# samuelkriegerbonini-dev/AstroBurst

Hardware: AMD Instinct MI355X
Metric: MPix/s sigma-clipped stack+stretch, 64x4096x4096 f32 (higher is better)
Workload: dtype f32

## Files before the change

### astroburst_amd/csrc/resample.hip

```cpp
#include "ab_common.hpp"
#include <algorithm>
#include <climits>
#include <cmath>

namespace {

__device__ __forceinline__ double cr_inner(double t) { return t * t * (1.5 * t - 2.5) + 1.0; }
__device__ __forceinline__ double cr_outer(double t) { return t * (t * (2.5 - 0.5 * t) - 4.0) + 2.0; }

__device__ __forceinline__ void catmull_weights(double f, double &w0, double &w1, double &w2, double &w3) {
    w0 = cr_outer(fabs(f + 1.0));
    w1 = cr_inner(fabs(f));
    w2 = cr_inner(fabs(f - 1.0));
    w3 = cr_outer(fabs(f - 2.0));
}

__device__ __forceinline__ int clamp_i32(int idx, int len) {
    return idx < 0 ? 0 : (idx >= len ? len - 1 : idx);
}

__device__ __forceinline__ float bicubic_taps(const float *__restrict__ src, int rows, int cols, int ld, int ix, int iy,
                                              double wx0, double wx1, double wx2, double wx3, double wy0, double wy1,
                                              double wy2, double wy3) {
    const int c0 = clamp_i32(ix - 1, cols), c1 = clamp_i32(ix, cols), c2 = clamp_i32(ix + 1, cols),
              c3 = clamp_i32(ix + 2, cols);
    const int r0 = clamp_i32(iy - 1, rows) * ld, r1 = clamp_i32(iy, rows) * ld, r2 = clamp_i32(iy + 1, rows) * ld,
              r3 = clamp_i32(iy + 2, rows) * ld;
    const double wy[4] = {wy0, wy1, wy2, wy3};
    const int rr[4] = {r0, r1, r2, r3};
    double val = 0.0;
#pragma unroll
    for (int j = 0; j < 4; ++j) {
        const float *row = src + rr[j];
        double row_val = (double)row[c0] * wx0;
        row_val += (double)row[c1] * wx1;
        row_val += (double)row[c2] * wx2;
        row_val += (double)row[c3] * wx3;
        const double t = row_val * wy[j];
        val = (j == 0) ? t : val + t;
    }
    return (float)val;
}

__device__ __forceinline__ float bicubic_taps_interior(const float *__restrict__ src, int ld, int ix, int iy, double wx0, double wx1,
                                                       double wx2, double wx3, double wy0, double wy1, double wy2, double wy3) {
    const float *p = src + (iy - 1) * ld + (ix - 1);
    const double wy[4] = {wy0, wy1, wy2, wy3};
    double val = 0.0;
#pragma unroll
    for (int j = 0; j < 4; ++j) {
        const float *row = p + j * ld;
        double row_val = (double)row[0] * wx0;
        row_val += (double)row[1] * wx1;
        row_val += (double)row[2] * wx2;
        row_val += (double)row[3] * wx3;
        const double t = row_val * wy[j];
        val = (j == 0) ? t : val + t;
    }
    return (float)val;
}

template <bool GUARD = false>
__device__ __forceinline__ float bicubic_sample(const float *__restrict__ src, int rows, int cols, int ld, double y, double x,
                                                bool sample = true) {
    const double xf = floor(x), yf = floor(y);
    double wx0, wx1, wx2, wx3, wy0, wy1, wy2, wy3;
    catmull_weights(x - xf, wx0, wx1, wx2, wx3);
    catmull_weights(y - yf, wy0, wy1, wy2, wy3);
    int ix = (int)xf, iy = (int)yf;
    if constexpr (GUARD) {
        if (x != x) ix = 0, wx0 = wx1 = wx2 = wx3 = 0.0;
        if (y != y) iy = 0, wy0 = wy1 = wy2 = wy3 = 0.0;
    }
    const bool interior = ix >= 1 && ix + 2 < cols && iy >= 1 && iy + 2 < rows;
    if (__all(interior || !sample)) {
        if (!sample) return 0.0f;
        return bicubic_taps_interior(src, ld, ix, iy, wx0, wx1, wx2, wx3, wy0, wy1, wy2, wy3);
    }
    if (!sample) return 0.0f;
    return bicubic_taps(src, rows, cols, ld, ix, iy, wx0, wx1, wx2, wx3, wy0, wy1, wy2, wy3);
}

__device__ __forceinline__ void xcd_band_piece(unsigned int &piece_x, unsigned int &piece_y) {
    piece_x = blockIdx.x;
    piece_y = blockIdx.y;
#ifndef AB_WARP_ROW_MAJOR
    if ((gridDim.x & 7u) != 0) {
        const unsigned int gx = gridDim.x, total = gx * gridDim.y, id = blockIdx.y * gx + blockIdx.x;
        const unsigned int c = id & 7u, k = id >> 3;
        unsigned int start = 0;
        for (unsigned int j = 0; j < c; ++j) start += (total - j + 7u) >> 3;
        const unsigned int t = start + k;
        piece_y = t / gx;
        piece_x = t - piece_y * gx;
    }
#endif
}

template <bool GUARD>
__global__ __launch_bounds__(256) void shift_kernel(const float *__restrict__ src, int rows, int cols, int ld, double dy,
                                                    double dx, float *__restrict__ out) {
    unsigned int piece_x, piece_y;
    xcd_band_piece(piece_x, piece_y);
    const int x = piece_x * 256 + threadIdx.x;
    const int y = piece_y;
    if (x >= cols) return;
    const double sy = (double)y + dy;
    const double sx = (double)x + dx;
    float r = 0.0f;
    if (!(sy < -0.5 || sy > (double)rows - 0.5 || sx < -0.5 || sx > (double)cols - 0.5))
        r = bicubic_sample<GUARD>(src, rows, cols, ld, sy, sx);
    out[(size_t)y * cols + x] = r;
}

__device__ __forceinline__ double cr_outer_fused(double t) { return t * (t * __builtin_fma(-0.5, t, 2.5) - 4.0) + 2.0; }
__device__ __forceinline__ void catmull_weights_fused(double f, double &w0, double &w1, double &w2, double &w3) {
    w0 = cr_outer_fused(fabs(f + 1.0));
    w1 = cr_inner(fabs(f));
    w2 = cr_inner(fabs(f - 1.0));
    w3 = cr_outer_fused(fabs(f - 2.0));
}

template <bool GUARD, bool NOLOAD = false, bool NOCVT = false>
__global__ __launch_bounds__(256) void warp_kernel(const float *__restrict__ src, int src_rows, int src_cols, double a,
                                                   double b, double tx, double c, double d, double ty, int out_rows,
                                                   int out_cols, float *__restrict__ out, int row0) {
#ifdef AB_WARP_WAVE_PRIO
    __builtin_amdgcn_s_setprio(AB_WARP_WAVE_PRIO);
#endif
    unsigned int piece_x, piece_y;
    xcd_band_piece(piece_x, piece_y);
    const int x0 = piece_x * 512 + threadIdx.x;
    const int y = piece_y + row0;
    const double yf = (double)y;
    float r[2];
    bool live[2];
#pragma unroll
    for (int u = 0; u < 2; ++u) {
        const int x = x0 + 256 * u;
        live[u] = x < out_cols;
        const double xf = (double)x;
        const double sx = a * xf + b * yf + tx;
        const double sy = c * xf + d * yf + ty;
        const double fx = floor(sx), fy = floor(sy);
        int ix, iy;
        asm("v_cvt_i32_f64 %0, %1" : "=v"(ix) : "v"(fx));
        asm("v_cvt_i32_f64 %0, %1" : "=v"(iy) : "v"(fy));
        bool in = live[u] && (unsigned)ix < (unsigned)(src_cols - 1) && (unsigned)iy < (unsigned)(src_rows - 1);
        if constexpr (GUARD) in = in && sx == sx && sy == sy;
        double wx0, wx1, wx2, wx3, wy0, wy1, wy2, wy3;
        catmull_weights_fused(sx - fx, wx0, wx1, wx2, wx3);
        catmull_weights_fused(sy - fy, wy0, wy1, wy2, wy3);
        const bool interior = ix >= 1 && ix + 2 < src_cols && iy >= 1 && iy + 2 < src_rows;
        r[u] = 0.0f;
        if constexpr (NOLOAD) {
            double val = 0.0;
            const double wy[4] = {wy0, wy1, wy2, wy3};
#pragma unroll
            for (int j = 0; j < 4; ++j) {
                float s0 = __int_as_float(0x3f800000 | ((ix + 4 * j) & 0xffff)), s1 = __int_as_float(0x3f800000 | ((ix + 4 * j + 1) & 0xffff)),
                      s2 = __int_as_float(0x3f800000 | ((iy + 4 * j + 2) & 0xffff)), s3 = __int_as_float(0x3f800000 | ((iy + 4 * j + 3) & 0xffff));
                double d0 = (double)s0, d1 = (double)s1, d2 = (double)s2, d3 = (double)s3;
                if constexpr (NOCVT) {
                    d0 = __longlong_as_double(0x3ff0000000000000ll | (long long)(unsigned)(ix + 4 * j));
                    d1 = __longlong_as_double(0x3ff0000000000000ll | (long long)(unsigned)(ix + 4 * j + 1));
                    d2 = __longlong_as_double(0x3ff0000000000000ll | (long long)(unsigned)(iy + 4 * j + 2));
                    d3 = __longlong_as_double(0x3ff0000000000000ll | (long long)(unsigned)(iy + 4 * j + 3));
                }
                double row_val = d0 * wx0;
                row_val += d1 * wx1;
                row_val += d2 * wx2;
                row_val += d3 * wx3;
                const double t = row_val * wy[j];
                val = (j == 0) ? t : val + t;
            }
            r[u] = in ? (float)val : 0.0f;
        } else if (__all(interior || !in)) {
            if (in) r[u] = bicubic_taps_interior(src, src_cols, ix, iy, wx0, wx1, wx2, wx3, wy0, wy1, wy2, wy3);
        } else if (in) {
            r[u] = bicubic_taps(src, src_rows, src_cols, src_cols, ix, iy, wx0, wx1, wx2, wx3, wy0, wy1, wy2, wy3);
        }
    }
#pragma unroll
    for (int u = 0; u < 2; ++u)
        if (live[u]) out[(size_t)piece_y * out_cols + x0 + 256 * u] = r[u];
}

__global__ __launch_bounds__(256) void resample_kernel(const float *__restrict__ src, int src_rows, int src_cols, double scale_y,
                                                       double scale_x, double half_shift_y, double half_shift_x, int out_cols,
                                                       float *__restrict__ out) {
    unsigned int piece_x, piece_y;
    xcd_band_piece(piece_x, piece_y);
    const int x = piece_x * 256 + threadIdx.x;
    const int y = piece_y;
    if (x >= out_cols) return;
    const double sy = (double)y * scale_y + half_shift_y;
    const double sx = (double)x * scale_x + half_shift_x;
    out[(size_t)y * out_cols + x] = bicubic_sample(src, src_rows, src_cols, src_cols, sy, sx);
}

}

int ab_resample_device(ab_ctx *ctx, const float *src, int64_t src_rows, int64_t src_cols, int64_t out_rows, int64_t out_cols,
                       float *out) {
    AB_HIP(ctx, hipSetDevice(ctx->device));
    if (out_rows == 0 || out_cols == 0) return ab_set_error(ctx, AB_ERR_INVALID, "Target dimensions must be > 0");
    if (out_rows == src_rows && out_cols == src_cols) {
        if (src != out) AB_HIP(ctx, hipMemcpyAsync(out, src, (size_t)src_rows * src_cols * sizeof(float), hipMemcpyDeviceToDevice, ctx->stream));
        return AB_OK;
    }
    AB_CHECK(ctx, src != out, "resample_image cannot run in place");
    AB_CHECK(ctx, src_rows > 0 && src_cols > 0, "resample_image: empty source");
    AB_CHECK(ctx, out_rows <= 65535 && out_rows * out_cols < (int64_t(1) << 31) && src_rows * src_cols < (int64_t(1) << 31),
             "image of %lld x %lld needs a tiled launch (not in this build)", (long long)out_rows, (long long)out_cols);
    const double scale_y = (double)src_rows / (double)out_rows, scale_x = (double)src_cols / (double)out_cols;
    const dim3 grid((unsigned)((out_cols + 255) / 256), (unsigned)out_rows), block(256);
    hipLaunchKernelGGL(resample_kernel, grid, block, 0, ctx->stream, src, (int)src_rows, (int)src_cols, scale_y, scale_x,
                       (scale_y - 1.0) * 0.5, (scale_x - 1.0) * 0.5, (int)out_cols, out);
    AB_HIP(ctx, hipGetLastError());
    return AB_OK;
}

int ab_shift_device(ab_ctx *ctx, const float *src, int64_t rows, int64_t cols, int64_t src_ld, double dy, double dx, float *out) {
    AB_HIP(ctx, hipSetDevice(ctx->device));
    if (fabs(dy) < 1e-12 && fabs(dx) < 1e-12) {
        if (src != out)
            AB_HIP(ctx, hipMemcpy2DAsync(out, cols * sizeof(float), src, src_ld * sizeof(float), cols * sizeof(float), rows,
                                         hipMemcpyDeviceToDevice, ctx->stream));
        return AB_OK;
    }
    AB_CHECK(ctx, src != out, "shift_image_subpixel cannot run in place");
    AB_CHECK(ctx, rows <= 65535 && rows * src_ld < (int64_t(1) << 31),
             "image of %lld x %lld needs a tiled launch (not in this build)", (long long)rows, (long long)cols);
    const dim3 grid((unsigned)((cols + 255) / 256), (unsigned)rows), block(256);
    if (std::isfinite(dy) && std::isfinite(dx))
        hipLaunchKernelGGL(shift_kernel<false>, grid, block, 0, ctx->stream, src, (int)rows, (int)cols, (int)src_ld, dy, dx, out);
    else
        hipLaunchKernelGGL(shift_kernel<true>, grid, block, 0, ctx->stream, src, (int)rows, (int)cols, (int)src_ld, dy, dx, out);
    AB_HIP(ctx, hipGetLastError());
    return AB_OK;
}

int ab_warp_device(ab_ctx *ctx, const float *src, int64_t src_rows, int64_t src_cols, const double t[6], int64_t out_rows,
                   int64_t out_cols, float *out) {
    return ab_warp_rows_device(ctx, src, src_rows, src_cols, t, out_rows, out_cols, 0, out_rows, out);
}

constexpr long kWarpLdsKB = 0;
int ab_warp_rows_device(ab_ctx *ctx, const float *src, int64_t src_rows, int64_t src_cols, const double t[6], int64_t out_rows,
                        int64_t out_cols, int64_t row0, int64_t nrows, float *out) {
    AB_HIP(ctx, hipSetDevice(ctx->device));
    AB_CHECK(ctx, row0 >= 0 && nrows >= 0 && row0 + nrows <= out_rows, "row band [%lld, %lld) leaves the %lld output rows", (long long)row0,
             (long long)(row0 + nrows), (long long)out_rows);
    if (nrows == 0) return AB_OK;
    AB_CHECK(ctx, src != out, "warp_image cannot run in place");
    AB_CHECK(ctx, out_rows <= 65535 && out_rows * out_cols < (int64_t(1) << 31) && src_rows * src_cols < (int64_t(1) << 31),
             "image of %lld x %lld needs a tiled launch (not in this build)", (long long)out_rows, (long long)out_cols);
    const dim3 grid((unsigned)((out_cols + 511) / 512), (unsigned)nrows), block(256);
#ifdef AB_DEV_ABLATION
    static const int ablate = ab_dev_env("AB_ABLATE_WARP") ? atoi(ab_dev_env("AB_ABLATE_WARP")) : 0;
    if (ablate == 1) return AB_OK;
    if (ablate == 3) {
        const dim3 g2((unsigned)((out_cols + 511) / 512), (unsigned)nrows);
        hipLaunchKernelGGL((warp_kernel<false, true, true>), g2, dim3(256), 0, ctx->stream, src, (int)src_rows, (int)src_cols, t[0], t[1], t[2], t[3],
                           t[4], t[5], (int)out_rows, (int)out_cols, out, (int)row0);
        return AB_OK;
    }
    if (ablate == 2) {
        const dim3 g2((unsigned)((out_cols + 511) / 512), (unsigned)nrows);
        hipLaunchKernelGGL((warp_kernel<false, true>), g2, dim3(256), 0, ctx->stream, src, (int)src_rows, (int)src_cols, t[0], t[1], t[2], t[3],
                           t[4], t[5], (int)out_rows, (int)out_cols, out, (int)row0);
        return AB_OK;
    }
#endif
    bool tame = true;
    for (int i = 0; i < 6; ++i) tame = tame && std::isfinite(t[i]) && fabs(t[i]) <= 1e150;
    static const unsigned warp_lds = [] {
        const char *e = ab_dev_env("AB_WARP_LDS_KB");
        const long kb = e ? atol(e) : kWarpLdsKB;
        return (unsigned)(kb < 0 ? 0 : (kb > 64 ? 64 : kb)) * 1024u;
    }();
    if (tame)
        hipLaunchKernelGGL(warp_kernel<false>, grid, block, warp_lds, ctx->stream, src, (int)src_rows, (int)src_cols, t[0], t[1], t[2], t[3],
                           t[4], t[5], (int)out_rows, (int)out_cols, out, (int)row0);
    else
        hipLaunchKernelGGL(warp_kernel<true>, grid, block, warp_lds, ctx->stream, src, (int)src_rows, (int)src_cols, t[0], t[1], t[2], t[3],
                           t[4], t[5], (int)out_rows, (int)out_cols, out, (int)row0);
    AB_HIP(ctx, hipGetLastError());
    return AB_OK;
}

extern "C" {

int ab_shift_image_subpixel(ab_ctx *ctx, const ab_plane *src, double dy, double dx, ab_plane_mut *out) try {
    if (!ctx) return AB_ERR_INVALID;
    AB_CHECK(ctx, src && out, "null plane");
    AB_CHECK(ctx, src->rows == out->rows && src->cols == out->cols, "shift_image_subpixel keeps the image dims");
    StagedPlane in;
    AB_TRY(ab_stage_in(ctx, src, &in));
    StagedOut so;
    int rc = ab_stage_out_begin(ctx, out, &so);
    if (rc == AB_OK) {
        rc = ab_shift_device(ctx, in.dptr, in.rows, in.cols, in.cols, dy, dx, so.dptr);
        if (rc == AB_OK)
            rc = ab_stage_out_finish(ctx, &so);
        else
            ab_stage_out_abort(ctx, &so);
    }
    ab_stage_release(ctx, &in);
    return rc;
} AB_CATCH(ctx)

int ab_warp_image_rows(ab_ctx *ctx, const ab_plane *src, const double transform[6], int64_t out_rows, int64_t row0, ab_plane_mut *out_band) try {
    if (!ctx) return AB_ERR_INVALID;
    AB_CHECK(ctx, src && out_band && transform && src->data && out_band->data, "null plane or transform");
    AB_CHECK(ctx, src->on_device && out_band->on_device, "ab_warp_image_rows takes device-resident planes");
    return ab_warp_rows_device(ctx, src->data, src->rows, src->cols, transform, out_rows, out_band->cols, row0, out_band->rows, out_band->data);
} AB_CATCH(ctx)

static void warp_source_rows(const double t[6], int64_t src_rows, int64_t src_cols, int64_t out_cols, int64_t row0, int64_t nrows,
                             int64_t *s0, int64_t *sn) {
    *s0 = 0;
    *sn = 0;
    if (nrows <= 0 || out_cols <= 0 || src_rows < 2 || src_cols < 2) return;
    for (int i = 0; i < 6; ++i)
        if (!std::isfinite(t[i]) || fabs(t[i]) > 1e150) {
            *sn = src_rows;
            return;
        }
    double lo = INFINITY, hi = -INFINITY;
    const double xs[2] = {0.0, (double)(out_cols - 1)}, ys[2] = {(double)row0, (double)(row0 + nrows - 1)};
    for (double xf : xs)
        for (double yf : ys) {
            const double sy = t[3] * xf + t[4] * yf + t[5];
            lo = std::min(lo, sy);
            hi = std::max(hi, sy);
        }
    const double last = (double)(src_rows - 2);
    if (!(hi >= 0.0) || !(floor(lo) <= last)) return;
    const int64_t f_lo = (int64_t)std::max(floor(lo), 0.0), f_hi = (int64_t)std::min(floor(hi), last);
    const int64_t a = std::max<int64_t>(f_lo - 1, 0), b = std::min<int64_t>(f_hi + 2, src_rows - 1);
    *s0 = a;
    *sn = b - a + 1;
}

int ab_warp_source_rows(const double transform[6], int64_t src_rows, int64_t src_cols, int64_t out_cols, int64_t row0, int64_t nrows,
                        int64_t *src_row0, int64_t *src_nrows) try {
    if (!transform || !src_row0 || !src_nrows || src_rows < 0 || src_cols < 0 || row0 < 0 || nrows < 0) return AB_ERR_INVALID;
    warp_source_rows(transform, src_rows, src_cols, out_cols, row0, nrows, src_row0, src_nrows);
    return AB_OK;
} AB_CATCH_NOCTX

int ab_shard_source_rows(const double *transforms, size_t n, int64_t src_rows, int64_t src_cols, int64_t out_rows, int64_t out_cols, int nranks,
                         int rank, int64_t *src_row0, int64_t *src_nrows) try {
    if ((!transforms && n) || !src_row0 || !src_nrows) return AB_ERR_INVALID;
    int64_t row0 = 0, nrows = 0;
    if (ab_shard_rows(out_rows, nranks, rank, &row0, &nrows) != AB_OK) return AB_ERR_INVALID;
    int64_t lo = INT64_MAX, hi = INT64_MIN;
    for (size_t i = 0; i < n; ++i) {
        int64_t s0 = 0, sn = 0;
        warp_source_rows(transforms + 6 * i, src_rows, src_cols, out_cols, row0, nrows, &s0, &sn);
        if (sn > 0) {
            lo = std::min(lo, s0);
            hi = std::max(hi, s0 + sn);
        }
    }
    *src_row0 = lo <= hi ? lo : 0;
    *src_nrows = lo <= hi ? hi - lo : 0;
    return AB_OK;
} AB_CATCH_NOCTX

int ab_warp_image_rows_from_band(ab_ctx *ctx, const ab_plane *src_band, int64_t src_row0, int64_t src_rows, const double transform[6],
                                 int64_t out_rows, int64_t row0, ab_plane_mut *out_band) try {
    if (!ctx) return AB_ERR_INVALID;
    AB_CHECK(ctx, src_band && out_band && transform && (out_band->rows == 0 || out_band->data), "null plane or transform");
    AB_CHECK(ctx, src_row0 >= 0 && src_band->rows >= 0 && src_row0 + src_band->rows <= src_rows, "source band [%lld, %lld) leaves the frame's %lld rows",
             (long long)src_row0, (long long)(src_row0 + src_band->rows), (long long)src_rows);
    if (out_band->rows == 0) return AB_OK;
    AB_CHECK(ctx, out_band->on_device && (src_band->rows == 0 || (src_band->data && src_band->on_device)), "ab_warp_image_rows_from_band takes device-resident planes");
    int64_t need0 = 0, need_n = 0;
    warp_source_rows(transform, src_rows, src_band->cols, out_band->cols, row0, out_band->rows, &need0, &need_n);
    AB_CHECK(ctx, need_n == 0 || (need0 >= src_row0 && need0 + need_n <= src_row0 + src_band->rows),
             "output rows [%lld, %lld) read source rows [%lld, %lld); the band holds [%lld, %lld)", (long long)row0, (long long)(row0 + out_band->rows),
             (long long)need0, (long long)(need0 + need_n), (long long)src_row0, (long long)(src_row0 + src_band->rows));
    const float *base = src_band->data ? src_band->data - src_row0 * src_band->cols : nullptr;
    if (!base) {
        base = out_band->data + 1;
    }
    return ab_warp_rows_device(ctx, base, src_rows, src_band->cols, transform, out_rows, out_band->cols, row0, out_band->rows, out_band->data);
} AB_CATCH(ctx)

int ab_warp_image(ab_ctx *ctx, const ab_plane *src, const double transform[6], ab_plane_mut *out) try {
    if (!ctx) return AB_ERR_INVALID;
    AB_CHECK(ctx, src && out && transform, "null plane or transform");
    StagedPlane in;
    AB_TRY(ab_stage_in(ctx, src, &in));
    StagedOut so;
    int rc = ab_stage_out_begin(ctx, out, &so);
    if (rc == AB_OK) {
        rc = ab_warp_device(ctx, in.dptr, in.rows, in.cols, transform, out->rows, out->cols, so.dptr);
        if (rc == AB_OK)
            rc = ab_stage_out_finish(ctx, &so);
        else
            ab_stage_out_abort(ctx, &so);
    }
    ab_stage_release(ctx, &in);
    return rc;
} AB_CATCH(ctx)

int ab_resample_image(ab_ctx *ctx, const ab_plane *src, ab_plane_mut *out) try {
    if (!ctx) return AB_ERR_INVALID;
    AB_CHECK(ctx, src && out, "null plane");
    if (out->rows == 0 || out->cols == 0) return ab_set_error(ctx, AB_ERR_INVALID, "Target dimensions must be > 0");
    StagedPlane in;
    AB_TRY(ab_stage_in(ctx, src, &in));
    StagedOut so;
    int rc = ab_stage_out_begin(ctx, out, &so);
    if (rc == AB_OK) {
        rc = ab_resample_device(ctx, in.dptr, in.rows, in.cols, out->rows, out->cols, so.dptr);
        if (rc == AB_OK)
            rc = ab_stage_out_finish(ctx, &so);
        else
            ab_stage_out_abort(ctx, &so);
    }
    ab_stage_release(ctx, &in);
    return rc;
} AB_CATCH(ctx)

}
```

Measured before the change: 112,300.

## Add multi-row warp kernel that shares source tap rows across adjacent outputs

Adds a warp kernel variant in which each thread computes K vertically adjacent output rows. When the affine map is close to identity in y, those outputs read overlapping 4x4 source neighbourhoods, so the kernel loads K+3 source rows once instead of 4K. The variant is selected when the transform is tame and near-unit in y, with a wave-uniform fallback to the per-pixel path. The intent is to cut redundant global loads and index math, at the cost of more registers per thread and fewer threads in the grid.

```diff
diff --git a/astroburst_amd/csrc/resample.hip b/astroburst_amd/csrc/resample.hip
--- a/astroburst_amd/csrc/resample.hip
+++ b/astroburst_amd/csrc/resample.hip
@@ -186,6 +186,99 @@
         if (live[u]) out[(size_t)piece_y * out_cols + x0 + 256 * u] = r[u];
 }
 
+template <int J>
+__device__ __forceinline__ double catmull_weight_fused(double f) {
+    if constexpr (J == 0) return cr_outer_fused(fabs(f + 1.0));
+    if constexpr (J == 1) return cr_inner(fabs(f));
+    if constexpr (J == 2) return cr_inner(fabs(f - 1.0));
+    return cr_outer_fused(fabs(f - 2.0));
+}
+
+template <int K>
+__global__ __launch_bounds__(256) void warp_kernel_shared(const float *__restrict__ src, int src_rows, int src_cols, double a, double b,
+                                                          double tx, double c, double d, double ty, int out_rows, int out_cols,
+                                                          float *__restrict__ out, int row0, int nrows) {
+    unsigned int piece_x, piece_y;
+    xcd_band_piece(piece_x, piece_y);
+    const int x = piece_x * 256 + threadIdx.x;
+    const int yb = piece_y * K;
+    const bool col_live = x < out_cols;
+    const double xf = (double)x;
+    const double axf = a * xf, cxf = c * xf;
+    int ix[K], iy[K];
+    double frx[K], fry[K];
+    bool in[K], live[K];
+    bool share = true;
+#pragma unroll
+    for (int k = 0; k < K; ++k) {
+        const double yf = (double)(yb + k + row0);
+        const double sx = axf + b * yf + tx;
+        const double sy = cxf + d * yf + ty;
+        const double fx = floor(sx), fy = floor(sy);
+        asm("v_cvt_i32_f64 %0, %1" : "=v"(ix[k]) : "v"(fx));
+        asm("v_cvt_i32_f64 %0, %1" : "=v"(iy[k]) : "v"(fy));
+        live[k] = col_live && yb + k < nrows;
+        in[k] = live[k] && (unsigned)ix[k] < (unsigned)(src_cols - 1) && (unsigned)iy[k] < (unsigned)(src_rows - 1);
+        frx[k] = sx - fx;
+        fry[k] = sy - fy;
+        const bool interior = ix[k] >= 1 && ix[k] + 2 < src_cols && iy[k] >= 1 && iy[k] + 2 < src_rows;
+        share = share && in[k] && interior && ix[k] == ix[0] && iy[k] == iy[0] + k;
+    }
+    float r[K];
+    if (__all(share)) {
+        const float *p = src + (iy[0] - 1) * src_cols + (ix[0] - 1);
+        double wx[K][4], val[K];
+#pragma unroll
+        for (int s = 0; s < K + 3; ++s) {
+            const float *row = p + s * src_cols;
+            const double t0 = (double)row[0], t1 = (double)row[1], t2 = (double)row[2], t3 = (double)row[3];
+#pragma unroll
+            for (int k = 0; k < K; ++k) {
+                const int j = s - k;
+                if (j < 0 || j > 3) continue;
+                if (j == 0) catmull_weights_fused(frx[k], wx[k][0], wx[k][1], wx[k][2], wx[k][3]);
+                double row_val = t0 * wx[k][0];
+                row_val += t1 * wx[k][1];
+                row_val += t2 * wx[k][2];
+                row_val += t3 * wx[k][3];
+                const double wy = j == 0 ? catmull_weight_fused<0>(fry[k])
+                                : j == 1 ? catmull_weight_fused<1>(fry[k])
+                                : j == 2 ? catmull_weight_fused<2>(fry[k])
+                                         : catmull_weight_fused<3>(fry[k]);
+                const double t = row_val * wy;
+                val[k] = (j == 0) ? t : val[k] + t;
+            }
+        }
+#pragma unroll
+        for (int k = 0; k < K; ++k) r[k] = (float)val[k];
+    } else {
+#pragma unroll
+        for (int k = 0; k < K; ++k) {
+            double wx0, wx1, wx2, wx3, wy0, wy1, wy2, wy3;
+            catmull_weights_fused(frx[k], wx0, wx1, wx2, wx3);
+            catmull_weights_fused(fry[k], wy0, wy1, wy2, wy3);
+            const bool interior = ix[k] >= 1 && ix[k] + 2 < src_cols && iy[k] >= 1 && iy[k] + 2 < src_rows;
+            r[k] = 0.0f;
+            if (__all(interior || !in[k])) {
+                if (in[k]) r[k] = bicubic_taps_interior(src, src_cols, ix[k], iy[k], wx0, wx1, wx2, wx3, wy0, wy1, wy2, wy3);
+            } else if (in[k]) {
+                r[k] = bicubic_taps(src, src_rows, src_cols, src_cols, ix[k], iy[k], wx0, wx1, wx2, wx3, wy0, wy1, wy2, wy3);
+            }
+        }
+    }
+#pragma unroll
+    for (int k = 0; k < K; ++k)
+        if (live[k]) out[(size_t)(yb + k) * out_cols + x] = r[k];
+}
+
+template <int K>
+void launch_warp_shared(ab_ctx *ctx, unsigned lds, const float *src, int64_t src_rows, int64_t src_cols, const double t[6], int64_t out_rows,
+                        int64_t out_cols, int64_t row0, int64_t nrows, float *out) {
+    const dim3 grid((unsigned)((out_cols + 255) / 256), (unsigned)((nrows + K - 1) / K)), block(256);
+    hipLaunchKernelGGL(warp_kernel_shared<K>, grid, block, lds, ctx->stream, src, (int)src_rows, (int)src_cols, t[0], t[1], t[2], t[3], t[4],
+                       t[5], (int)out_rows, (int)out_cols, out, (int)row0, (int)nrows);
+}
+
 __global__ __launch_bounds__(256) void resample_kernel(const float *__restrict__ src, int src_rows, int src_cols, double scale_y,
                                                        double scale_x, double half_shift_y, double half_shift_x, int out_cols,
                                                        float *__restrict__ out) {
@@ -247,6 +340,7 @@
 }
 
 constexpr long kWarpLdsKB = 0;
+constexpr int kWarpShareK = 3;
 int ab_warp_rows_device(ab_ctx *ctx, const float *src, int64_t src_rows, int64_t src_cols, const double t[6], int64_t out_rows,
                         int64_t out_cols, int64_t row0, int64_t nrows, float *out) {
     AB_HIP(ctx, hipSetDevice(ctx->device));
@@ -280,12 +374,27 @@
         const long kb = e ? atol(e) : kWarpLdsKB;
         return (unsigned)(kb < 0 ? 0 : (kb > 64 ? 64 : kb)) * 1024u;
     }();
-    if (tame)
-        hipLaunchKernelGGL(warp_kernel<false>, grid, block, warp_lds, ctx->stream, src, (int)src_rows, (int)src_cols, t[0], t[1], t[2], t[3],
-                           t[4], t[5], (int)out_rows, (int)out_cols, out, (int)row0);
-    else
-        hipLaunchKernelGGL(warp_kernel<true>, grid, block, warp_lds, ctx->stream, src, (int)src_rows, (int)src_cols, t[0], t[1], t[2], t[3],
-                           t[4], t[5], (int)out_rows, (int)out_cols, out, (int)row0);
+    int share_k = tame && fabs(t[4] - 1.0) <= 1.0 / 64.0 && fabs(t[1]) <= 1.0 / 64.0 ? kWarpShareK : 0;
+#ifdef AB_DEV_ABLATION
+    static const int share_env = ab_dev_env("AB_WARP_SHARE_K") ? atoi(ab_dev_env("AB_WARP_SHARE_K")) : kWarpShareK;
+    if (share_k) share_k = share_env;
+#endif
+    switch (share_k) {
+#ifdef AB_DEV_ABLATION
+    case 2: launch_warp_shared<2>(ctx, warp_lds, src, src_rows, src_cols, t, out_rows, out_cols, row0, nrows, out); break;
+    case 3: launch_warp_shared<3>(ctx, warp_lds, src, src_rows, src_cols, t, out_rows, out_cols, row0, nrows, out); break;
+    case 4: launch_warp_shared<4>(ctx, warp_lds, src, src_rows, src_cols, t, out_rows, out_cols, row0, nrows, out); break;
+#else
+    case kWarpShareK: launch_warp_shared<kWarpShareK>(ctx, warp_lds, src, src_rows, src_cols, t, out_rows, out_cols, row0, nrows, out); break;
+#endif
+    default:
+        if (tame)
+            hipLaunchKernelGGL(warp_kernel<false>, grid, block, warp_lds, ctx->stream, src, (int)src_rows, (int)src_cols, t[0], t[1], t[2], t[3],
+                               t[4], t[5], (int)out_rows, (int)out_cols, out, (int)row0);
+        else
+            hipLaunchKernelGGL(warp_kernel<true>, grid, block, warp_lds, ctx->stream, src, (int)src_rows, (int)src_cols, t[0], t[1], t[2], t[3],
+                               t[4], t[5], (int)out_rows, (int)out_cols, out, (int)row0);
+    }
     AB_HIP(ctx, hipGetLastError());
     return AB_OK;
 }
```

New measurement: 114,000 (median of 6 runs). +1.5%, better.
